# bayesiains/nflows

Hardware: AMD Instinct MI355X
Metric: log_prob samples/sec (dim=64, K=8, 32-layer RQ-NSF) + max |fwd∘inv − x| (higher is better)
Workload: dtype f32 (inputs, outputs, spline arithmetic, accumulation; conditioner GEMMs: every fp32 operand carried as 3 f16 pieces = 33 significand bits, i.e. at the reference's own fp32 operand width, 5 cross products per multiply-add -- 3 on the f16 MFMA, the 2 at the 2^-22 level from the pieces' high bytes on

## Files before the change

### nflows_amd/csrc/f16x3_gemm.hpp

```cpp
#pragma once

#include "bf16x3_gemm.hpp"

namespace nfa {

typedef _Float16 f16x8 __attribute__((ext_vector_type(8)));
typedef int i32x8 __attribute__((ext_vector_type(8)));

namespace k8x {

constexpr int kScaleA = 119, kScaleB = 127;

#ifdef NFA_ABL_NO_MFMA
#define NFA_K8X_F16(a, b, c) (c)
#define NFA_K8X_BF8(a, b, c) (c)
#else
#define NFA_K8X_F16(a, b, c) __builtin_amdgcn_mfma_f32_32x32x16_f16(a, b, c, 0, 0, 0)
#define NFA_K8X_BF8(a, b, c) __builtin_amdgcn_mfma_scale_f32_32x32x64_f8f6f4(a, b, c, 1, 1, 0, kScaleA, 0, kScaleB)
#endif

__device__ __forceinline__ void request_stage(WeightStream& sm) {
    const int dst_slot = sm.slot >= 1 ? sm.slot - 1 : kRing - 1;
    const char* stage = reinterpret_cast<const char*>(sm.w) + (size_t)sm.fetch * (kStageVec4 * 16);
    const __amdgpu_buffer_rsrc_t rsrc =
        __builtin_amdgcn_make_buffer_rsrc(const_cast<char*>(stage), (short)0, kStageVec4 * 16, 0x00020000);
    const int wave = __builtin_amdgcn_readfirstlane(sm.tid >> 6);
    char* slot = reinterpret_cast<char*>(sm.ring) + dst_slot * (kStageVec4 * 16) + wave * (kWave * 16);
    const unsigned lane_off = (unsigned)sm.tid * 16u;
#pragma unroll
    for (int i = 0; i < 3; ++i)
        __builtin_amdgcn_raw_ptr_buffer_load_lds(rsrc, (__attribute__((address_space(3))) void*)(slot + i * kBlock * 16), 16,
                                                 lane_off, i * kBlock * 16, 0, 0);
    sm.fetch = (sm.fetch + 1 == sm.num_stages) ? 0 : sm.fetch + 1;
}

struct Pieces {
    uvec4 h, l, r;
};

#define NFA_K8X_ASM asm volatile

#define NFA_K8X_SPLIT_REST                                                  \
    "v_fma_mixlo_f16 %1, %3, 1.0, 0 op_sel_hi:[0,0,0]\n\t"                  \
    "v_fma_mixhi_f16 %1, %4, 1.0, 0 op_sel_hi:[0,0,0]\n\t"                  \
    "v_fma_mix_f32 %3, %3, 1.0, -%1 op_sel_hi:[0,0,1]\n\t"                  \
    "v_fma_mix_f32 %4, %4, 1.0, -%1 op_sel:[0,0,1] op_sel_hi:[0,0,1]\n\t"   \
    "v_fma_mixlo_f16 %2, %3, %8, 0 op_sel_hi:[0,0,0]\n\t"                   \
    "v_fma_mixhi_f16 %2, %4, %8, 0 op_sel_hi:[0,0,0]"
template <bool RELU = false>
__device__ __forceinline__ void split3_scaled(float v0, float v1, float scale, unsigned& hi, unsigned& lo, unsigned& rr) {
#if defined(NFA_K8X_NO_ASM)
    typedef _Float16 h2 __attribute__((ext_vector_type(2)));
    if (RELU) {
        v0 = __builtin_isnan(v0) ? v0 : (v0 > 0.0f ? v0 : 0.0f);
        v1 = __builtin_isnan(v1) ? v1 : (v1 > 0.0f ? v1 : 0.0f);
    }
    const float x0 = v0 * scale, x1 = v1 * scale;
    const h2 h = {(_Float16)x0, (_Float16)x1};
    const float t0 = x0 - (float)h[0], t1 = x1 - (float)h[1];
    const h2 l = {(_Float16)t0, (_Float16)t1};
    const h2 r = {(_Float16)((t0 - (float)l[0]) * 256.0f), (_Float16)((t1 - (float)l[1]) * 256.0f)};
    hi = __builtin_bit_cast(unsigned, h);
    lo = __builtin_bit_cast(unsigned, l);
    rr = __builtin_bit_cast(unsigned, r);
#else
    unsigned h, l, r;
    float t0, t1;
    if constexpr (RELU)
        NFA_K8X_ASM(
            "v_maximum3_f32 %3, %5, 0, 0\n\t"
            "v_maximum3_f32 %4, %6, 0, 0\n\t"
            "v_fma_mixlo_f16 %0, %3, %7, 0 op_sel_hi:[0,0,0]\n\t"
            "v_fma_mixhi_f16 %0, %4, %7, 0 op_sel_hi:[0,0,0]\n\t"
            "v_fma_mix_f32 %3, %3, %7, -%0 op_sel_hi:[0,0,1]\n\t"
            "v_fma_mix_f32 %4, %4, %7, -%0 op_sel:[0,0,1] op_sel_hi:[0,0,1]\n\t"
            NFA_K8X_SPLIT_REST
            : "=&v"(h), "=&v"(l), "=&v"(r), "=&v"(t0), "=&v"(t1)
            : "v"(v0), "v"(v1), "v"(scale), "s"(256.0f));
    else
        NFA_K8X_ASM(
            "v_fma_mixlo_f16 %0, %5, %7, 0 op_sel_hi:[0,0,0]\n\t"
            "v_fma_mixhi_f16 %0, %6, %7, 0 op_sel_hi:[0,0,0]\n\t"
            "v_fma_mix_f32 %3, %5, %7, -%0 op_sel_hi:[0,0,1]\n\t"
            "v_fma_mix_f32 %4, %6, %7, -%0 op_sel:[0,0,1] op_sel_hi:[0,0,1]\n\t"
            NFA_K8X_SPLIT_REST
            : "=&v"(h), "=&v"(l), "=&v"(r), "=&v"(t0), "=&v"(t1)
            : "v"(v0), "v"(v1), "v"(scale), "s"(256.0f));
    hi = h;
    lo = l;
    rr = r;
#endif
}
#undef NFA_K8X_SPLIT_REST

__device__ __forceinline__ i32x8 bf8_operand(const Pieces& p0, const Pieces& p1) {
    constexpr unsigned kHigh = 0x07050301u;
    i32x8 b;
    b[0] = (int)__builtin_amdgcn_perm(p0.r[1], p0.r[0], kHigh);
    b[1] = (int)__builtin_amdgcn_perm(p0.r[3], p0.r[2], kHigh);
    b[2] = (int)__builtin_amdgcn_perm(p0.h[1], p0.h[0], kHigh);
    b[3] = (int)__builtin_amdgcn_perm(p0.h[3], p0.h[2], kHigh);
    b[4] = (int)__builtin_amdgcn_perm(p1.r[1], p1.r[0], kHigh);
    b[5] = (int)__builtin_amdgcn_perm(p1.r[3], p1.r[2], kHigh);
    b[6] = (int)__builtin_amdgcn_perm(p1.h[1], p1.h[0], kHigh);
    b[7] = (int)__builtin_amdgcn_perm(p1.h[3], p1.h[2], kHigh);
    return b;
}

template <bool RELU, bool WB = true>
__device__ __forceinline__ void tile_to_pieces(const f32x16& a, float scale, Pieces& p0, Pieces& p1) {
    if constexpr (WB) asm volatile("s_nop 7\n\ts_nop 3" : : "v"(a));
#pragma unroll
    for (int q2 = 0; q2 < 8; ++q2) {
        unsigned h, l, r;
        split3_scaled<RELU>(a[q2 * 2], a[q2 * 2 + 1], scale, h, l, r);
        if (q2 < 4) {
            p0.h[q2] = h;
            p0.l[q2] = l;
            p0.r[q2] = r;
        } else {
            p1.h[q2 - 4] = h;
            p1.l[q2 - 4] = l;
            p1.r[q2 - 4] = r;
        }
    }
}

__device__ __forceinline__ i32x8 join_x(vec4f lo, vec4f hi) {
    const uvec4 a = __builtin_bit_cast(uvec4, lo), b = __builtin_bit_cast(uvec4, hi);
    return i32x8{(int)a[0], (int)a[1], (int)a[2], (int)a[3], (int)b[0], (int)b[1], (int)b[2], (int)b[3]};
}

struct Lead {
    vec4f h0, l0, h1, l1;
};
__device__ __forceinline__ Lead read_lead(const vec4f* stage) {
    return Lead{stage[0 * 64], stage[1 * 64], stage[2 * 64], stage[3 * 64]};
}

#define NFA_K8X_FENCE() __builtin_amdgcn_sched_barrier(0)

template <bool LAST>
__device__ __forceinline__ void stage_kmajor(f32x16& acc0, f32x16& acc1, const Pieces& b0, const Pieces& b1, const i32x8& bx,
                                             WeightStream& sm, int lane, Lead& lead) {
    request_stage(sm);
    const vec4f* cur = sm.ring + sm.slot * kStageVec4 + lane;
    const f16x8 bh0 = __builtin_bit_cast(f16x8, b0.h), bl0 = __builtin_bit_cast(f16x8, b0.l);
    const f16x8 bh1 = __builtin_bit_cast(f16x8, b1.h), bl1 = __builtin_bit_cast(f16x8, b1.l);
    const vec4f x0l = cur[4 * 64], x0h = cur[5 * 64];
    const vec4f h0 = cur[6 * 64], l0 = cur[7 * 64], h1 = cur[8 * 64], l1 = cur[9 * 64], x1l = cur[10 * 64], x1h = cur[11 * 64];
    NFA_K8X_FENCE();
    {
        const f16x8 ah0 = __builtin_bit_cast(f16x8, lead.h0), al0 = __builtin_bit_cast(f16x8, lead.l0);
        const f16x8 ah1 = __builtin_bit_cast(f16x8, lead.h1), al1 = __builtin_bit_cast(f16x8, lead.l1);
        acc0 = NFA_K8X_F16(ah0, bl0, acc0);
        acc0 = NFA_K8X_F16(al0, bh0, acc0);
        acc0 = NFA_K8X_F16(ah0, bh0, acc0);
        acc0 = NFA_K8X_F16(ah1, bl1, acc0);
        acc0 = NFA_K8X_F16(al1, bh1, acc0);
        acc0 = NFA_K8X_F16(ah1, bh1, acc0);
        acc0 = NFA_K8X_BF8(join_x(x0l, x0h), bx, acc0);
    }
    const f16x8 ah0 = __builtin_bit_cast(f16x8, h0), al0 = __builtin_bit_cast(f16x8, l0);
    const f16x8 ah1 = __builtin_bit_cast(f16x8, h1), al1 = __builtin_bit_cast(f16x8, l1);
    const i32x8 ax = join_x(x1l, x1h);
    acc1 = NFA_K8X_F16(ah0, bl0, acc1);
    acc1 = NFA_K8X_F16(al0, bh0, acc1);
    acc1 = NFA_K8X_F16(ah0, bh0, acc1);
    NFA_K8X_FENCE();
    stream_advance(sm);
    if constexpr (!LAST) lead = read_lead(sm.ring + sm.slot * kStageVec4 + lane);
    NFA_K8X_FENCE();
    acc1 = NFA_K8X_F16(ah1, bl1, acc1);
    acc1 = NFA_K8X_F16(al1, bh1, acc1);
    acc1 = NFA_K8X_F16(ah1, bh1, acc1);
    acc1 = NFA_K8X_BF8(ax, bx, acc1);
}

template <int NKS, class PairFn>
__device__ __forceinline__ void gemm_kmajor_pairs(f32x16 (&acc)[4], WeightStream& sm, int lane, PairFn&& pair) {
    static_assert(NKS % 2 == 0, "pairs of k-steps");
    Lead lead = read_lead(sm.ring + sm.slot * kStageVec4 + lane);
#pragma unroll
    for (int pr = 0; pr < NKS / 2; ++pr) {
        Pieces b0, b1;
        pair(pr, b0, b1);
        const i32x8 bx = bf8_operand(b0, b1);
        stage_kmajor<false>(acc[0], acc[1], b0, b1, bx, sm, lane, lead);
        if (pr + 1 < NKS / 2) stage_kmajor<false>(acc[2], acc[3], b0, b1, bx, sm, lane, lead);
        else stage_kmajor<true>(acc[2], acc[3], b0, b1, bx, sm, lane, lead);
    }
}

template <int NKS>
__device__ __forceinline__ void gemm_kmajor(f32x16 (&acc)[4], const Pieces (&p)[8], WeightStream& sm, int lane) {
    gemm_kmajor_pairs<NKS>(acc, sm, lane, [&](int pr, Pieces& b0, Pieces& b1) {
        b0 = p[2 * pr];
        b1 = p[2 * pr + 1];
    });
}

__device__ __forceinline__ void gemm_kmajor_relu(f32x16 (&acc)[4], const f32x16 (&src)[4], float scale, WeightStream& sm,
                                                 int lane) {
    gemm_kmajor_pairs<8>(acc, sm, lane, [&](int pr, Pieces& b0, Pieces& b1) {
        if (pr == 0) tile_to_pieces<true, true>(src[pr], scale, b0, b1);
        else tile_to_pieces<true, false>(src[pr], scale, b0, b1);
    });
}

}
}
```

### nflows_amd/csrc/rqs_resnet_f16x3_kernel.hpp

```cpp
#pragma once

#include "f16x3_gemm.hpp"
#include "rqs_resnet_f16_kernel.hpp"

#include <hip/hip_ext.h>
#include <stdlib.h>
#include <type_traits>

namespace nfa {
namespace k8x {

struct Args {
    const float* x;
    const vec4f* w;
    const float* bias;
    const float* scales;
    const int32_t* tables;
    float* out;
    float* lad;
    int32_t* redo;
    int32_t* status;
    int64_t batch;
    int D, dt, di, num_blocks, num_layers, num_stages, bias_per_layer, accumulate;
    RqsDev sp;
    int normal, skip_out;
    float log_z, act_scale;
    int Ds;
    float* dbg_logits;
};

typedef __attribute__((address_space(3))) float lds_f32;
typedef __attribute__((address_space(3))) int lds_i32;

using nfa::load_bias_tile;

__device__ __forceinline__ void load_bias_tile(f32x16& acc, const lds_f32* bias_tile_half) {
    typedef __attribute__((address_space(3))) const vec4f lds_vec4f;
    lds_vec4f* bp = reinterpret_cast<lds_vec4f*>(bias_tile_half);
#pragma unroll
    for (int q4 = 0; q4 < 4; ++q4) {
        const vec4f b = bp[q4];
        acc[q4 * 4 + 0] = b.x;
        acc[q4 * 4 + 1] = b.y;
        acc[q4 * 4 + 2] = b.z;
        acc[q4 * 4 + 3] = b.w;
    }
}

template <int BYTES>
__device__ __forceinline__ void bias_area_piece(const void* src, int src_bytes, int piece_off, lds_f32* dst) {
    const __amdgpu_buffer_rsrc_t rsrc = __builtin_amdgcn_make_buffer_rsrc(
        const_cast<char*>(static_cast<const char*>(src) + piece_off), (short)0, src_bytes - piece_off, 0x00020000);
    unsigned all = ~0u;
    asm volatile("" : "+s"(all));
    const unsigned lane = __builtin_amdgcn_mbcnt_hi(all, __builtin_amdgcn_mbcnt_lo(all, 0u));
    static_assert(BYTES == 16 || BYTES == 4, "dwordx4 or dword pieces");
    if constexpr (BYTES == 16)
        __builtin_amdgcn_raw_ptr_buffer_load_lds(rsrc, (__attribute__((address_space(3))) void*)dst, 16, lane * 16, 0, 0, 0);
    else
        __builtin_amdgcn_raw_ptr_buffer_load_lds(rsrc, (__attribute__((address_space(3))) void*)dst, 4, lane * 4, 0, 0, 0);
}
__host__ __device__ constexpr int bias_area_hidden_floats(int num_blocks) { return 128 + 256 * num_blocks; }
__host__ __device__ constexpr int bias_area_final_floats(int final_floats) { return (final_floats + 255) & ~255; }
__host__ __device__ constexpr int bias_area_floats(int num_blocks, int final_floats) {
    return bias_area_hidden_floats(num_blocks) + kTabLayer + bias_area_final_floats(final_floats);
}

template <int N>
__device__ __forceinline__ void uniform_load(const float* p, float (&v)[N]) {
    static_assert(N == 2 || N == 4, "one or two pairs");
    uint64_t v01, v23 = 0;
    if constexpr (N == 2)
        asm volatile("s_load_dwordx2 %0, %1, 0x0\n\ts_waitcnt lgkmcnt(0)" : "=&s"(v01) : "s"(p) : "memory");
    else
        asm volatile("s_load_dwordx2 %0, %2, 0x0\n\ts_load_dwordx2 %1, %2, 0x8\n\ts_waitcnt lgkmcnt(0)"
                     : "=&s"(v01), "=&s"(v23) : "s"(p) : "memory");
    v[0] = __builtin_bit_cast(float, (unsigned)v01);
    v[1] = __builtin_bit_cast(float, (unsigned)(v01 >> 32));
    if constexpr (N == 4) {
        v[2] = __builtin_bit_cast(float, (unsigned)v23);
        v[3] = __builtin_bit_cast(float, (unsigned)(v23 >> 32));
    }
}

struct NoWeave {
    template <int U0, int U1>
    __device__ __forceinline__ void span() {}
};
template <int UNIT, class Steps>
struct UnitWeave {
    Steps &fa, &fb;
    const RqsDev& sp;
    template <int U0, int U1>
    __device__ __forceinline__ void span() {
        constexpr int N = k8h::spline_unit_slices<UNIT, Steps>();
        k8h::spline_unit_range<UNIT, (U0 * N) / 32, (U1 * N) / 32>(fa, fb, sp);
    }
};
template <int MASK, class Steps>
struct SeqWeave {
    Steps& f;
    const RqsDev& sp;
    template <int U0, int U1>
    __device__ __forceinline__ void span() {
        constexpr int N = k8h::spline_seq_count<MASK, Steps>();
        k8h::spline_seq_range<MASK, (U0 * N) / 32, (U1 * N) / 32>(f, sp);
    }
};

#define NFA_K8X_PUMP_F16(U, A_, B_)                                         \
    acc = NFA_K8X_F16(A_, B_, acc);                                         \
    __builtin_amdgcn_sched_barrier(0);                                      \
    w.template span<(U), (U) + 1>();                                        \
    __builtin_amdgcn_sched_barrier(0)
#define NFA_K8X_PUMP_BF8(U, A_, B_)                                         \
    acc = NFA_K8X_BF8(A_, B_, acc);                                         \
    __builtin_amdgcn_sched_barrier(0);                                      \
    w.template span<(U), (U) + 2>();                                        \
    __builtin_amdgcn_sched_barrier(0)

template <int HS, class W>
__device__ __forceinline__ void stage_pumped(f32x16& acc, const Pieces (&p)[8], const i32x8 (&bx)[4], WeightStream& sm, int lane,
                                             Lead& lead, W& w) {
    request_stage(sm);
    const vec4f* cur = sm.ring + sm.slot * kStageVec4 + lane;
    vec4f xa = cur[8 * 64], xb = cur[9 * 64];
    vec4f fh0 = lead.h0, fl0 = lead.l0, fh1 = lead.h1, fl1 = lead.l1;
    {
        const Pieces& b0 = p[HS * 4 + 0];
        const Pieces& b1 = p[HS * 4 + 1];
        const f16x8 bh0 = __builtin_bit_cast(f16x8, b0.h), bl0 = __builtin_bit_cast(f16x8, b0.l);
        const f16x8 bh1 = __builtin_bit_cast(f16x8, b1.h), bl1 = __builtin_bit_cast(f16x8, b1.l);
        const f16x8 ah0 = __builtin_bit_cast(f16x8, fh0), al0 = __builtin_bit_cast(f16x8, fl0);
        const f16x8 ah1 = __builtin_bit_cast(f16x8, fh1), al1 = __builtin_bit_cast(f16x8, fl1);
        const i32x8 ax = join_x(xa, xb);
        NFA_K8X_PUMP_F16(HS * 16 + 0, ah0, bl0);
        NFA_K8X_PUMP_F16(HS * 16 + 1, al0, bh0);
        NFA_K8X_PUMP_F16(HS * 16 + 2, ah0, bh0);
        fh0 = cur[4 * 64];
        fl0 = cur[5 * 64];
        NFA_K8X_PUMP_F16(HS * 16 + 3, ah1, bl1);
        NFA_K8X_PUMP_F16(HS * 16 + 4, al1, bh1);
        NFA_K8X_PUMP_F16(HS * 16 + 5, ah1, bh1);
        fh1 = cur[6 * 64];
        fl1 = cur[7 * 64];
        NFA_K8X_PUMP_BF8(HS * 16 + 6, ax, bx[HS * 2 + 0]);
        xa = cur[10 * 64];
        xb = cur[11 * 64];
    }
    {
        const Pieces& b0 = p[HS * 4 + 2];
        const Pieces& b1 = p[HS * 4 + 3];
        const f16x8 bh0 = __builtin_bit_cast(f16x8, b0.h), bl0 = __builtin_bit_cast(f16x8, b0.l);
        const f16x8 bh1 = __builtin_bit_cast(f16x8, b1.h), bl1 = __builtin_bit_cast(f16x8, b1.l);
        const f16x8 ah0 = __builtin_bit_cast(f16x8, fh0), al0 = __builtin_bit_cast(f16x8, fl0);
        const f16x8 ah1 = __builtin_bit_cast(f16x8, fh1), al1 = __builtin_bit_cast(f16x8, fl1);
        const i32x8 ax = join_x(xa, xb);
        NFA_K8X_PUMP_F16(HS * 16 + 8, ah0, bl0);
        NFA_K8X_PUMP_F16(HS * 16 + 9, al0, bh0);
        NFA_K8X_PUMP_F16(HS * 16 + 10, ah0, bh0);
        NFA_K8X_PUMP_F16(HS * 16 + 11, ah1, bl1);
        NFA_K8X_PUMP_F16(HS * 16 + 12, al1, bh1);
        NFA_K8X_PUMP_F16(HS * 16 + 13, ah1, bh1);
        stream_advance(sm);
        lead = read_lead(sm.ring + sm.slot * kStageVec4 + lane);
        __builtin_amdgcn_sched_barrier(0);
        NFA_K8X_PUMP_BF8(HS * 16 + 14, ax, bx[HS * 2 + 1]);
    }
}
#undef NFA_K8X_PUMP_F16
#undef NFA_K8X_PUMP_BF8

template <class W>
__device__ __forceinline__ void gemm_tile_pumped(f32x16& acc, const Pieces (&p)[8], const i32x8 (&bx)[4], WeightStream& sm, int lane,
                                                 Lead& lead, W&& w) {
    stage_pumped<0>(acc, p, bx, sm, lane, lead, w);
    stage_pumped<1>(acc, p, bx, sm, lane, lead, w);
}

template <int TI, int T, int KB, class Steps, class BiasPtr>
__device__ __forceinline__ void any_group_tiles(f32x16& acc, Steps& f, BiasPtr gb, const Pieces (&p)[8], const i32x8 (&bx)[4],
                                                WeightStream& sm, int lane, Lead& lead, const RqsDev& sp) {
    if constexpr (TI < T) {
        constexpr int kMask = k8h::any_tile_mask(KB, TI);
        load_bias_tile(acc, gb + TI * 32);
        if constexpr (kMask != 0) gemm_tile_pumped(acc, p, bx, sm, lane, lead, SeqWeave<kMask, Steps>{f, sp});
        else gemm_tile_pumped(acc, p, bx, sm, lane, lead, NoWeave{});
        k8h::take_chunk<TI, KB>(f, acc);
        any_group_tiles<TI + 1, T, KB, Steps, BiasPtr>(acc, f, gb, p, bx, sm, lane, lead, sp);
    }
}

__device__ __forceinline__ bool not_finite(float v) { return !(__builtin_fabsf(v) < INFINITY); }

template <bool INVERSE, int INIT_KS, bool DBG, int KB, bool BIAS_LDS>
__device__ __forceinline__ void rqs_resnet_f16x3_body(const Args& a) {
    static_assert(!DBG || KB == 8, "the diagnostic instances: 8 bins");
    constexpr int kFinalRows = KB == 8 ? 24 : 16 * ((3 * KB - 1 + 15) / 16);
    constexpr int NW = kBlock / kWave;
    extern __shared__ __attribute__((aligned(16))) float lds_dyn[];
    __shared__ int s_tab[2][kTabLayer];
    __shared__ int s_final[128];
    __shared__ int s_bad[NW];
    const int tid = threadIdx.x, lane = tid & 63, wave = __builtin_amdgcn_readfirstlane(tid >> 6);
    const int D = a.D, dt = a.dt;
    int my_status = 0;
    auto checked = [&](int v, bool used) {
        my_status |= (used && (v < 0 || v >= D)) ? NFA_STATUS_BAD_INDEX : 0;
        return v < 0 ? 0 : (v >= D ? D - 1 : v);
    };
    const int te = tid & (kTabLayer - 1);
    s_tab[0][te] = checked(a.tables[te], te < kTabTr ? te < a.di : te - kTabTr < dt);
    s_final[te] = checked(a.tables[a.num_layers * kTabLayer + te], te < D);

    WeightStream sm;
    sm.w = a.w;
    sm.ring = reinterpret_cast<vec4f*>(lds_dyn);
    sm.slot = 1;
    sm.fetch = 0;
    sm.num_stages = a.num_stages * a.num_layers;
    sm.tid = tid;
    lds_f32* s_area = (lds_f32*)lds_dyn + kRing * kStageVec4 * 4 + NW * D * kRowPad;
    lds_f32* s_traw = s_area + bias_area_hidden_floats(a.num_blocks);
    auto request_hidden = [&](int layer) {
        const float* src = a.bias + (size_t)layer * a.bias_per_layer;
        const int bytes = bias_area_hidden_floats(a.num_blocks) * 4;
        if (wave >= 2) bias_area_piece<4>(src, bytes, (wave - 2) * 256, s_area + (wave - 2) * 64);
        for (int j = wave; j < a.num_blocks; j += NW) bias_area_piece<16>(src, bytes, 512 + j * 1024, s_area + 128 + j * 256);
    };
    if constexpr (BIAS_LDS) request_hidden(0);
    request_stage(sm);
    sm.slot = 2;
    request_stage(sm);
    sm.slot = 0;
    asm volatile("s_waitcnt vmcnt(0)" ::: "memory");
    __syncthreads();

#ifdef NFA_K8X_STAGGER
    if (blockIdx.x >= (gridDim.x >> 1))
        for (int i = 0; i < NFA_K8X_STAGGER; ++i) __builtin_amdgcn_s_sleep(127);
#endif
    lds_f32* s_row = (lds_f32*)lds_dyn + kRing * kStageVec4 * 4 + wave * D * kRowPad;
    lds_f32* s_fbias = BIAS_LDS ? s_traw + kTabLayer : s_area;
    auto request_final = [&](int layer) {
        const float* src = a.bias + (size_t)layer * a.bias_per_layer + bias_area_hidden_floats(a.num_blocks);
        const int bytes = dt * kFinalRows * 4;
        for (int j = wave; j * 1024 < bytes; j += NW) bias_area_piece<16>(src, bytes, j * 1024, s_fbias + j * 256);
    };
    auto request_table = [&](int layer) {
        if (wave < 2) bias_area_piece<4>(a.tables + layer * kTabLayer, kTabLayer * 4, wave * 256, s_traw + wave * 64);
    };
    const int groups = dt >> 2;
    const int64_t num_quads = a.batch >> 7;
    const int gemms = 2 + 2 * a.num_blocks;
    const float S = a.act_scale;
    int tb = 0;

    for (int64_t quad = blockIdx.x; quad < num_quads; quad += gridDim.x) {
        const int64_t row0 = (quad << 7) + (wave << 5);
        int lane_here = lane, di = a.di;
        asm volatile("" : "+v"(lane_here), "+s"(di));
        const int half = lane_here >> 5, r = lane_here & 31;
        {
            const vec4f* xv = reinterpret_cast<const vec4f*>(a.x + row0 * D);
            const int nvec = D * 8;
            for (int e0 = lane; e0 < nvec; e0 += kWave * 4) {
                vec4f v[4];
#pragma unroll
                for (int u = 0; u < 4; ++u) {
                    const int e = e0 + u * kWave;
                    v[u] = xv[e < nvec ? e : 0];
                }
#pragma unroll
                for (int u = 0; u < 4; ++u) {
                    const int e = e0 + u * kWave;
                    if (e < nvec) {
                        const int rr = (e * 4) / D, c0 = e * 4 - rr * D;
                        s_row[(c0 + 0) * kRowPad + rr] = v[u].x;
                        s_row[(c0 + 1) * kRowPad + rr] = v[u].y;
                        s_row[(c0 + 2) * kRowPad + rr] = v[u].z;
                        s_row[(c0 + 3) * kRowPad + rr] = v[u].w;
                    }
                }
            }
        }
        __builtin_amdgcn_fence(__ATOMIC_RELEASE, "wavefront");
        __builtin_amdgcn_fence(__ATOMIC_ACQUIRE, "wavefront");

        float lad_acc = 0.0f;
        int quad_status = 0;
        for (int layer = 0; layer < a.num_layers; ++layer) {
            if ((layer + (blockIdx.x >= (gridDim.x >> 1) ? 1 : 0)) & 1) __builtin_amdgcn_s_setprio(1);
            else __builtin_amdgcn_s_setprio(0);
            const int* tab = s_tab[tb];
            const int nl = layer + 1 < a.num_layers ? layer + 1 : 0;
            if constexpr (!BIAS_LDS) {
                unsigned all = ~0u;
                asm volatile("" : "+s"(all));
                const int te_l = (int)__builtin_amdgcn_mbcnt_hi(all, __builtin_amdgcn_mbcnt_lo(all, 0u)) + ((wave & 1) << 6);
                s_tab[tb ^ 1][te_l] = checked(a.tables[nl * kTabLayer + te_l], te_l < kTabTr ? te_l < a.di : te_l - kTabTr < dt);
            }
            if constexpr (BIAS_LDS) {
                request_final(layer);
                request_table(nl);
                __builtin_amdgcn_sched_barrier(0);
            }
            std::conditional_t<BIAS_LDS, const lds_f32*, const float*> bias;
            if constexpr (BIAS_LDS) bias = s_area + half * 16;
            else bias = a.bias + (size_t)layer * a.bias_per_layer + half * 16;
            const float* sc = a.scales + (size_t)layer * gemms * 2;
            Pieces p[8];

#pragma unroll
            for (int ks = 0; ks < INIT_KS; ++ks) {
#pragma unroll
                for (int j2 = 0; j2 < 4; ++j2) {
                    const int i0 = ks * 16 + half * 8 + j2 * 2;
                    float v0 = s_row[tab[kTabId + i0] * kRowPad + r], v1 = s_row[tab[kTabId + i0 + 1] * kRowPad + r];
                    v0 = i0 < di ? v0 : 0.0f;
                    v1 = i0 + 1 < di ? v1 : 0.0f;
                    unsigned hi, lo, rr;
                    split3_scaled(v0, v1, S, hi, lo, rr);
                    p[ks].h[j2] = hi;
                    p[ks].l[j2] = lo;
                    p[ks].r[j2] = rr;
                }
            }

            f32x16 h[4];
            float hs;
            {
#pragma unroll
                for (int t = 0; t < 4; ++t) load_bias_tile(h[t], bias + t * 32);
                gemm_kmajor<INIT_KS>(h, p, sm, lane);
                float s0[2];
                uniform_load(sc, s0);
                hs = s0[0];
            }
            bias += 128;
            sc += 2;
            if constexpr (BIAS_LDS) {
                unsigned all = ~0u;
                asm volatile("" : "+s"(all));
                const int te_l = (int)__builtin_amdgcn_mbcnt_hi(all, __builtin_amdgcn_mbcnt_lo(all, 0u)) + ((wave & 1) << 6);
                s_tab[tb ^ 1][te_l] = checked(((const lds_i32*)s_traw)[te_l], te_l < kTabTr ? te_l < a.di : te_l - kTabTr < dt);
            } else {
                const float* fbias = a.bias + (size_t)layer * a.bias_per_layer + 128 + 256 * a.num_blocks;
                for (int i = tid; i < dt * kFinalRows; i += kBlock) s_fbias[i] = fbias[i];
                if (a.num_blocks == 0) __syncthreads();
            }

            for (int blk = 0; blk < a.num_blocks; ++blk) {
                float sb[4];
                f32x16 u[4];
#pragma unroll
                for (int t = 0; t < 4; ++t) load_bias_tile(u[t], bias + t * 32);
                gemm_kmajor_relu(u, h, hs, sm, lane);
                uniform_load(sc, sb);
                const float skip = hs * sb[3];
#pragma unroll
                for (int t = 0; t < 4; ++t) {
                    f32x16 b1;
                    load_bias_tile(b1, bias + 128 + t * 32);
#pragma unroll
                    for (int q_ = 0; q_ < 16; ++q_) h[t][q_] = __builtin_fmaf(h[t][q_], skip, b1[q_]);
                }
                gemm_kmajor_relu(h, u, sb[0], sm, lane);
                hs = sb[2];
                bias += 256;
                sc += 4;
            }

            if constexpr (BIAS_LDS) {
                request_hidden(nl);
                __builtin_amdgcn_sched_barrier(0);
            }
#pragma unroll
            for (int t = 0; t < 4; ++t) tile_to_pieces<false>(h[t], hs, p[2 * t], p[2 * t + 1]);

            if constexpr (KB == 8) {
                using Steps = FusedSteps<INVERSE, 8>;
                Steps fa{}, fb{};
                float sf[2];
                uniform_load(sc, sf);
                const float kappa = sf[0];
                fa.kappa = fb.kappa = kappa;
                fa.kl2e = fb.kl2e = 1.44269502162933349609375f * kappa;
                fa.tail_s = fb.tail_s = a.sp.tail_logit * sf[1];
                lds_f32* slot_b = s_row;
                const lds_f32* fbias = s_fbias + half * 16;
                i32x8 bx[4];
#pragma unroll
                for (int j = 0; j < 4; ++j) bx[j] = bf8_operand(p[2 * j], p[2 * j + 1]);
                Lead lead = read_lead(sm.ring + sm.slot * kStageVec4 + lane);
                f32x16 acc[3];
                auto commit = [&](Steps& f, lds_f32* slot) {
                    *slot = f.y;
                    lad_acc += f.lad;
                    quad_status |= f.status;
                };
                [[maybe_unused]] auto store_logits = [&](const f32x16& t, int tile) {
                    if constexpr (DBG) {
                        if (layer == a.num_layers - 1) {
                            float* dst = a.dbg_logits + (size_t)(row0 + r) * (dt * kFinalRows) + tile * 32 + half * 16;
#pragma unroll
                            for (int q_ = 0; q_ < 16; ++q_) dst[q_] = t[q_] * kappa;
                            asm volatile("s_waitcnt vmcnt(0)" ::: "memory");
                        }
                    }
                };
                UnitWeave<k8h::kUnitNumA, Steps> w0{fa, fb, a.sp};
                UnitWeave<k8h::kUnitFinishA, Steps> w1{fa, fb, a.sp};
                UnitWeave<k8h::kUnitFinishB, Steps> w2{fa, fb, a.sp};
                for (int g = 0; g < groups; ++g) {
                    lds_f32* slot0 = s_row + tab[kTabTr + g * 4 + half * 2] * kRowPad + r;
                    lds_f32* slot1 = s_row + tab[kTabTr + g * 4 + half * 2 + 1] * kRowPad + r;
                    load_bias_tile(acc[0], fbias + (g * 3 + 0) * 32);
                    if (g > 0) {
                        gemm_tile_pumped(acc[0], p, bx, sm, lane, lead, w2);
                        commit(fb, slot_b);
                    } else {
                        gemm_tile_pumped(acc[0], p, bx, sm, lane, lead, NoWeave{});
                    }
                    store_logits(acc[0], g * 3 + 0);
                    fa.x = *slot0;
#pragma unroll
                    for (int j = 0; j < 8; ++j) {
                        fa.ew[j] = acc[0][j];
                        fa.eh[j] = acc[0][8 + j];
                    }
                    load_bias_tile(acc[1], fbias + (g * 3 + 1) * 32);
                    gemm_tile_pumped(acc[1], p, bx, sm, lane, lead, w0);
                    store_logits(acc[1], g * 3 + 1);
                    fb.x = *slot1;
#pragma unroll
                    for (int j = 0; j < 8; ++j) {
                        if (j < 7) fa.sd[j] = acc[1][j];
                        fb.ew[j] = acc[1][8 + j];
                    }
                    load_bias_tile(acc[2], fbias + (g * 3 + 2) * 32);
                    gemm_tile_pumped(acc[2], p, bx, sm, lane, lead, w1);
                    store_logits(acc[2], g * 3 + 2);
                    commit(fa, slot0);
#pragma unroll
                    for (int j = 0; j < 8; ++j) {
                        fb.eh[j] = acc[2][j];
                        if (j < 7) fb.sd[j] = acc[2][8 + j];
                    }
                    slot_b = slot1;
                }
                k8h::spline_unit_range<k8h::kUnitFinishB, 0, k8h::spline_unit_slices<k8h::kUnitFinishB, Steps>()>(fa, fb, a.sp);
                commit(fb, slot_b);
            }
            else {
                constexpr int T = kFinalRows / 16;
                static_assert(T >= 1 && T <= 6, "2 .. 32 bins");
                using Steps = FusedSteps<INVERSE, KB>;
                constexpr int kRest = k8h::any_rest_mask(KB);
                Steps f{};
                float sf[2];
                uniform_load(sc, sf);
                const float kappa = sf[0];
                f.kappa = kappa;
                f.kl2e = 1.44269502162933349609375f * kappa;
                f.tail_s = a.sp.tail_logit * sf[1];
                const lds_f32* fbias = s_fbias + half * 16;
                i32x8 bx[4];
#pragma unroll
                for (int j = 0; j < 4; ++j) bx[j] = bf8_operand(p[2 * j], p[2 * j + 1]);
                Lead lead = read_lead(sm.ring + sm.slot * kStageVec4 + lane);
                const int groups_any = dt >> 1;
                f32x16 acc;
                lds_f32* slot = s_row + tab[kTabTr + half] * kRowPad + r;
                load_bias_tile(acc, fbias);
                gemm_tile_pumped(acc, p, bx, sm, lane, lead, NoWeave{});
                for (int g = 0; g < groups_any; ++g) {
                    const lds_f32* gb = fbias + g * T * 32;
                    f.x = *slot;
                    k8h::take_chunk<0, KB>(f, acc);
                    any_group_tiles<1, T, KB, Steps>(acc, f, gb, p, bx, sm, lane, lead, a.sp);
                    if (g + 1 < groups_any) {
                        lds_f32* next_slot = s_row + tab[kTabTr + (g + 1) * 2 + half] * kRowPad + r;
                        load_bias_tile(acc, gb + T * 32);
                        gemm_tile_pumped(acc, p, bx, sm, lane, lead, SeqWeave<kRest, Steps>{f, a.sp});
                        *slot = f.y;
                        slot = next_slot;
                    } else {
                        k8h::spline_seq_range<kRest, 0, k8h::spline_seq_count<kRest, Steps>()>(f, a.sp);
                        *slot = f.y;
                    }
                    lad_acc += f.lad;
                    quad_status |= f.status;
                }
            }
            tb ^= 1;
            __builtin_amdgcn_fence(__ATOMIC_RELEASE, "wavefront");
            __builtin_amdgcn_fence(__ATOMIC_ACQUIRE, "wavefront");
        }

        lad_acc += __shfl_xor(lad_acc, 32, kWave);
        const float sumsq = tile_row_sumsq((const float*)s_row, a.Ds, half, r);
        const bool bad = not_finite(lad_acc) || not_finite(sumsq);
        const bool wave_bad = __builtin_amdgcn_ballot_w64(bad) != 0;
        if (lane == 0) s_bad[wave] = wave_bad ? 1 : 0;
        asm volatile("s_waitcnt vmcnt(0)" ::: "memory");
        __syncthreads();
        int any_bad = 0;
#pragma unroll
        for (int w_ = 0; w_ < NW; ++w_) any_bad |= s_bad[w_];
        if (!any_bad) {
            if (!a.skip_out) {
                vec4f* ov = reinterpret_cast<vec4f*>(a.out + row0 * D);
                const int nvec = D * 8;
                for (int e = lane; e < nvec; e += kWave) {
                    const int rr = (e * 4) / D, c0 = e * 4 - rr * D;
                    vec4f v;
                    v.x = s_row[s_final[c0 + 0] * kRowPad + rr];
                    v.y = s_row[s_final[c0 + 1] * kRowPad + rr];
                    v.z = s_row[s_final[c0 + 2] * kRowPad + rr];
                    v.w = s_row[s_final[c0 + 3] * kRowPad + rr];
                    ov[e] = v;
                }
            }
            if (half == 0) {
                float* dst = a.lad + row0 + r;
                float v = a.accumulate ? *dst + lad_acc : lad_acc;
                if (a.normal) v = (-0.5f * sumsq - a.log_z) + v;
                *dst = v;
            }
            my_status |= quad_status;
        }
        if (tid == 0) a.redo[quad] = any_bad ? 1 : 0;
        asm volatile("s_waitcnt vmcnt(0)" ::: "memory");
        __syncthreads();
    }
    asm volatile("s_waitcnt vmcnt(0)" ::: "memory");
    if (my_status && a.status) atomicOr(a.status, my_status);
}

template <bool INVERSE, int INIT_KS, bool DBG = false, int KB = 8>
__global__ void __launch_bounds__(kBlock, 2) rqs_resnet_f16x3_kernel(const Args a) {
    rqs_resnet_f16x3_body<INVERSE, INIT_KS, DBG, KB, true>(a);
}
template <bool INVERSE, int INIT_KS, bool DBG = false, int KB = 8>
__global__ void __launch_bounds__(kBlock, 2) rqs_resnet_f16x3_global_bias_kernel(const Args a) {
    rqs_resnet_f16x3_body<INVERSE, INIT_KS, DBG, KB, false>(a);
}

}
}


namespace nfa {
namespace k8x {
typedef void (*KernelFn)(const Args);
KernelFn bins_kernel_a(int K, bool inverse, int init_ks, bool bias_lds);
KernelFn bins_kernel_b(int K, bool inverse, int init_ks, bool bias_lds);
}
}
```

Measured before the change: 27.13 million.

## Reorder k-major stage MFMAs and weave next tile's fp32-to-f16x3 split between them

Rewrites the k-major GEMM stage so MFMAs are issued in source-B order, alternating between the two accumulators, with LDS reads of weight pieces spread between them. When the ReLU tile source is active (BIAS_LDS), it interleaves the per-slice split of the next k-pair's activations into f16 pieces between MFMAs instead of doing the whole conversion afterwards. The goal is to hide the VALU conversion work and LDS latency under MFMA execution. It adds many scheduling fences and extra register pressure from carrying the next pieces. An optional phase-priority mode is also added but is off by default.

```diff
diff --git a/nflows_amd/csrc/f16x3_gemm.hpp b/nflows_amd/csrc/f16x3_gemm.hpp
--- a/nflows_amd/csrc/f16x3_gemm.hpp
+++ b/nflows_amd/csrc/f16x3_gemm.hpp
@@ -1,6 +1,8 @@
 #pragma once
 
 #include "bf16x3_gemm.hpp"
+
+#include <type_traits>
 
 namespace nfa {
 
@@ -140,6 +142,197 @@
 
 #define NFA_K8X_FENCE() __builtin_amdgcn_sched_barrier(0)
 
+#ifndef NFA_K8X_SRCB_ORDER
+#define NFA_K8X_SRCB_ORDER 1
+#endif
+#ifndef NFA_K8X_WEAVE
+#define NFA_K8X_WEAVE 1
+#endif
+#if NFA_K8X_WEAVE && !NFA_K8X_SRCB_ORDER
+#error "NFA_K8X_WEAVE needs NFA_K8X_SRCB_ORDER: the slices' register plan is the reordered stage's"
+#endif
+
+#if NFA_K8X_SRCB_ORDER
+
+struct KLead {
+    vec4f h0, g0, l0;
+};
+__device__ __forceinline__ KLead read_klead(const vec4f* stage) {
+    return KLead{stage[0 * 64], stage[6 * 64], stage[1 * 64]};
+}
+
+#define NFA_K8X_KEEP2(a_, b_) asm volatile("" : : "v"(a_), "v"(b_))
+#define NFA_K8X_KEEP5(a_, b_, c_, d_, e_) asm volatile("" : : "v"(a_), "v"(b_), "v"(c_), "v"(d_), "v"(e_))
+
+struct NoSlices {
+    static constexpr bool kActive = false;
+    template <int Q2>
+    __device__ __forceinline__ void slice() {}
+};
+template <bool RELU>
+struct TileSlices {
+    static constexpr bool kActive = true;
+    const f32x16& a;
+    float scale;
+    Pieces &p0, &p1;
+    template <int Q2>
+    __device__ __forceinline__ void slice() {
+        unsigned h, l, r;
+        split3_scaled<RELU>(a[Q2 * 2], a[Q2 * 2 + 1], scale, h, l, r);
+        Pieces& p = Q2 < 4 ? p0 : p1;
+        p.h[Q2 & 3] = h;
+        p.l[Q2 & 3] = l;
+        p.r[Q2 & 3] = r;
+    }
+};
+
+__host__ __device__ constexpr int kmajor_slice_at(int half, int k) {
+    return half == 0 ? (k == 5 ? 0 : k == 8 ? 1 : k == 11 ? 2 : k == 13 ? 3 : -1)
+                     : (k == 2 ? 4 : k == 5 ? 5 : k == 8 ? 6 : k == 11 ? 7 : -1);
+}
+template <int HALF, int K, class W>
+__device__ __forceinline__ void kmajor_slot(W& w) {
+    constexpr int kSlice = kmajor_slice_at(HALF, K);
+    if constexpr (W::kActive && kSlice >= 0) {
+        w.template slice<kSlice>();
+    }
+}
+template <int HALF, int K, class W>
+constexpr bool kmajor_slot_used() { return W::kActive && kmajor_slice_at(HALF, K) >= 0; }
+
+template <bool LAST, int HALF, bool MAKE_BX, class W>
+__device__ __forceinline__ void stage_kmajor(f32x16& acc0, f32x16& acc1, const Pieces& b0, const Pieces& b1, i32x8& bx,
+                                             WeightStream& sm, int lane, KLead& lead, W& w) {
+    request_stage(sm);
+    const vec4f* cur = sm.ring + sm.slot * kStageVec4 + lane;
+    const f16x8 bh0 = __builtin_bit_cast(f16x8, b0.h), bl0 = __builtin_bit_cast(f16x8, b0.l);
+    const f16x8 bh1 = __builtin_bit_cast(f16x8, b1.h), bl1 = __builtin_bit_cast(f16x8, b1.l);
+    const vec4f t0h0 = lead.h0, t1h0 = lead.g0, t0l0 = lead.l0;
+    const vec4f t1l0 = cur[7 * 64], t0h1 = cur[2 * 64], t1h1 = cur[8 * 64], t0l1 = cur[3 * 64];
+    NFA_K8X_FENCE();
+    acc0 = NFA_K8X_F16(__builtin_bit_cast(f16x8, t0h0), bl0, acc0);
+    NFA_K8X_FENCE();
+    acc1 = NFA_K8X_F16(__builtin_bit_cast(f16x8, t1h0), bl0, acc1);
+    NFA_K8X_FENCE();
+    if constexpr (MAKE_BX) bx = bf8_operand(b0, b1);
+    kmajor_slot<HALF, 2>(w);
+    NFA_K8X_FENCE();
+    acc0 = NFA_K8X_F16(__builtin_bit_cast(f16x8, t0l0), bh0, acc0);
+    NFA_K8X_FENCE();
+    acc1 = NFA_K8X_F16(__builtin_bit_cast(f16x8, t1l0), bh0, acc1);
+    NFA_K8X_FENCE();
+    const vec4f t1l1 = cur[9 * 64], x0l = cur[4 * 64];
+    NFA_K8X_FENCE();
+    acc0 = NFA_K8X_F16(__builtin_bit_cast(f16x8, t0h0), bh0, acc0);
+    NFA_K8X_FENCE();
+    kmajor_slot<HALF, 5>(w);
+    if constexpr (kmajor_slot_used<HALF, 5, W>()) NFA_K8X_KEEP2(t1l0, t0h0);
+    NFA_K8X_FENCE();
+    acc1 = NFA_K8X_F16(__builtin_bit_cast(f16x8, t1h0), bh0, acc1);
+    NFA_K8X_FENCE();
+    const vec4f x0h = cur[5 * 64], x1l = cur[10 * 64], x1h = cur[11 * 64];
+    NFA_K8X_FENCE();
+    acc0 = NFA_K8X_F16(__builtin_bit_cast(f16x8, t0h1), bl1, acc0);
+    NFA_K8X_FENCE();
+    acc1 = NFA_K8X_F16(__builtin_bit_cast(f16x8, t1h1), bl1, acc1);
+    NFA_K8X_FENCE();
+    kmajor_slot<HALF, 8>(w);
+    NFA_K8X_FENCE();
+    acc0 = NFA_K8X_F16(__builtin_bit_cast(f16x8, t0l1), bh1, acc0);
+    NFA_K8X_FENCE();
+    acc1 = NFA_K8X_F16(__builtin_bit_cast(f16x8, t1l1), bh1, acc1);
+    NFA_K8X_FENCE();
+    acc0 = NFA_K8X_F16(__builtin_bit_cast(f16x8, t0h1), bh1, acc0);
+    const i32x8 ax0 = join_x(x0l, x0h), ax1 = join_x(x1l, x1h);
+    NFA_K8X_FENCE();
+    kmajor_slot<HALF, 11>(w);
+    if constexpr (kmajor_slot_used<HALF, 11, W>()) NFA_K8X_KEEP2(t1l1, t0h1);
+    NFA_K8X_FENCE();
+    stream_advance(sm);
+    if constexpr (!LAST) lead = read_klead(sm.ring + sm.slot * kStageVec4 + lane);
+    NFA_K8X_FENCE();
+    acc1 = NFA_K8X_F16(__builtin_bit_cast(f16x8, t1h1), bh1, acc1);
+    NFA_K8X_FENCE();
+    acc0 = NFA_K8X_BF8(ax0, bx, acc0);
+    NFA_K8X_FENCE();
+    kmajor_slot<HALF, 13>(w);
+    if constexpr (kmajor_slot_used<HALF, 13, W>()) NFA_K8X_KEEP2(t1h1, ax0);
+    NFA_K8X_FENCE();
+    acc1 = NFA_K8X_BF8(ax1, bx, acc1);
+    NFA_K8X_FENCE();
+}
+
+template <int NKS, class Src>
+__device__ __forceinline__ void gemm_kmajor_pairs(f32x16 (&acc)[4], WeightStream& sm, int lane, Src&& src) {
+    static_assert(NKS % 2 == 0, "pairs of k-steps");
+    constexpr bool kWeave = std::remove_reference_t<Src>::kWeave;
+    KLead lead = read_klead(sm.ring + sm.slot * kStageVec4 + lane);
+    Pieces b0, b1;
+    src.pair(0, b0, b1);
+    i32x8 bx = bf8_operand(b0, b1);
+    NoSlices none;
+#pragma unroll
+    for (int pr = 0; pr < NKS / 2; ++pr) {
+        constexpr bool kWoven = kWeave;
+        Pieces n0, n1;
+        if (pr + 1 < NKS / 2) {
+            if constexpr (kWeave) {
+                auto w = src.slices(pr + 1, n0, n1);
+                if (pr == 0) stage_kmajor<false, 0, false>(acc[0], acc[1], b0, b1, bx, sm, lane, lead, w);
+                else stage_kmajor<false, 0, kWoven>(acc[0], acc[1], b0, b1, bx, sm, lane, lead, w);
+                stage_kmajor<false, 1, false>(acc[2], acc[3], b0, b1, bx, sm, lane, lead, w);
+                NFA_K8X_KEEP5(b0.h, b0.l, b1.h, b1.l, bx);
+                b0 = n0;
+                b1 = n1;
+            } else {
+                stage_kmajor<false, 0, false>(acc[0], acc[1], b0, b1, bx, sm, lane, lead, none);
+                stage_kmajor<false, 1, false>(acc[2], acc[3], b0, b1, bx, sm, lane, lead, none);
+                src.pair(pr + 1, b0, b1);
+                bx = bf8_operand(b0, b1);
+            }
+        } else {
+            if (pr == 0) stage_kmajor<false, 0, false>(acc[0], acc[1], b0, b1, bx, sm, lane, lead, none);
+            else stage_kmajor<false, 0, kWoven>(acc[0], acc[1], b0, b1, bx, sm, lane, lead, none);
+            stage_kmajor<true, 1, false>(acc[2], acc[3], b0, b1, bx, sm, lane, lead, none);
+        }
+    }
+}
+
+template <int NKS>
+struct PiecesSource {
+    static constexpr bool kWeave = false;
+    const Pieces (&p)[8];
+    __device__ __forceinline__ void pair(int pr, Pieces& b0, Pieces& b1) {
+        b0 = p[2 * pr];
+        b1 = p[2 * pr + 1];
+    }
+};
+template <int NKS>
+__device__ __forceinline__ void gemm_kmajor(f32x16 (&acc)[4], const Pieces (&p)[8], WeightStream& sm, int lane) {
+    gemm_kmajor_pairs<NKS>(acc, sm, lane, PiecesSource<NKS>{p});
+}
+
+template <bool WEAVE>
+struct ReluTileSource {
+    static constexpr bool kWeave = WEAVE && NFA_K8X_WEAVE != 0;
+    const f32x16 (&src)[4];
+    float scale;
+    __device__ __forceinline__ void pair(int pr, Pieces& b0, Pieces& b1) {
+        if (pr == 0) tile_to_pieces<true, true>(src[pr], scale, b0, b1);
+        else tile_to_pieces<true, false>(src[pr], scale, b0, b1);
+    }
+    __device__ __forceinline__ TileSlices<true> slices(int pr, Pieces& n0, Pieces& n1) {
+        return TileSlices<true>{src[pr], scale, n0, n1};
+    }
+};
+template <bool WEAVE = true>
+__device__ __forceinline__ void gemm_kmajor_relu(f32x16 (&acc)[4], const f32x16 (&src)[4], float scale, WeightStream& sm,
+                                                 int lane) {
+    gemm_kmajor_pairs<8>(acc, sm, lane, ReluTileSource<WEAVE>{src, scale});
+}
+
+#else
+
 template <bool LAST>
 __device__ __forceinline__ void stage_kmajor(f32x16& acc0, f32x16& acc1, const Pieces& b0, const Pieces& b1, const i32x8& bx,
                                              WeightStream& sm, int lane, Lead& lead) {
@@ -200,6 +393,7 @@
     });
 }
 
+template <bool WEAVE = false>
 __device__ __forceinline__ void gemm_kmajor_relu(f32x16 (&acc)[4], const f32x16 (&src)[4], float scale, WeightStream& sm,
                                                  int lane) {
     gemm_kmajor_pairs<8>(acc, sm, lane, [&](int pr, Pieces& b0, Pieces& b1) {
@@ -208,5 +402,7 @@
     });
 }
 
-}
-}
+#endif
+
+}
+}
diff --git a/nflows_amd/csrc/rqs_resnet_f16x3_kernel.hpp b/nflows_amd/csrc/rqs_resnet_f16x3_kernel.hpp
--- a/nflows_amd/csrc/rqs_resnet_f16x3_kernel.hpp
+++ b/nflows_amd/csrc/rqs_resnet_f16x3_kernel.hpp
@@ -6,6 +6,10 @@
 #include <hip/hip_ext.h>
 #include <stdlib.h>
 #include <type_traits>
+
+#ifndef NFA_K8X_PHASE_PRIO
+#define NFA_K8X_PHASE_PRIO 0
+#endif
 
 namespace nfa {
 namespace k8x {
@@ -290,8 +294,12 @@
         float lad_acc = 0.0f;
         int quad_status = 0;
         for (int layer = 0; layer < a.num_layers; ++layer) {
+#if NFA_K8X_PHASE_PRIO
+            __builtin_amdgcn_s_setprio(1);
+#else
             if ((layer + (blockIdx.x >= (gridDim.x >> 1) ? 1 : 0)) & 1) __builtin_amdgcn_s_setprio(1);
             else __builtin_amdgcn_s_setprio(0);
+#endif
             const int* tab = s_tab[tb];
             const int nl = layer + 1 < a.num_layers ? layer + 1 : 0;
             if constexpr (!BIAS_LDS) {
@@ -355,7 +363,7 @@
                 f32x16 u[4];
 #pragma unroll
                 for (int t = 0; t < 4; ++t) load_bias_tile(u[t], bias + t * 32);
-                gemm_kmajor_relu(u, h, hs, sm, lane);
+                gemm_kmajor_relu<BIAS_LDS>(u, h, hs, sm, lane);
                 uniform_load(sc, sb);
                 const float skip = hs * sb[3];
 #pragma unroll
@@ -365,7 +373,7 @@
 #pragma unroll
                     for (int q_ = 0; q_ < 16; ++q_) h[t][q_] = __builtin_fmaf(h[t][q_], skip, b1[q_]);
                 }
-                gemm_kmajor_relu(h, u, sb[0], sm, lane);
+                gemm_kmajor_relu<BIAS_LDS>(h, u, sb[0], sm, lane);
                 hs = sb[2];
                 bias += 256;
                 sc += 4;
@@ -375,6 +383,9 @@
                 request_hidden(nl);
                 __builtin_amdgcn_sched_barrier(0);
             }
+#if NFA_K8X_PHASE_PRIO
+            __builtin_amdgcn_s_setprio(0);
+#endif
 #pragma unroll
             for (int t = 0; t < 4; ++t) tile_to_pieces<false>(h[t], hs, p[2 * t], p[2 * t + 1]);
 
```

After: 27.29 million, median of 6. No clear change (+0.6%).
